# totgokhung123/Event-Retrival-In-Video-Learning-Transferable-Visual-Model-From-Supervised-Natural-Language

Measured on AMD Instinct MI355X. Metric: frames/sec embedded+ranked, ViT-B/32 224², 1/2/4/8 MI355X; R@1/5/10 parity, higher is better.
Workload: dtype bf16; 1 GPU; ViT-B/32 bf16, 10000 frames/GPU x 32 text queries, top-10 (BASELINE configs[1]); frames_per_gpu=10000, global_frames=10000, queries=32, k=10, image_chunk=10000, parallelism=dp1

## Files before the change

event-retrival-in-video-learning-transferable-visual-model-from-supervised-natural-language_amd/csrc/attention.hip:

```cpp
#include <algorithm>
#include <cstdlib>
#include <type_traits>

#include "common.hpp"
#include "internal.hpp"

namespace miclip {

namespace {


typedef short s16x4 __attribute__((ext_vector_type(4)));
typedef short s16x8 __attribute__((ext_vector_type(8)));

template <int V>
using Int = std::integral_constant<int, V>;

constexpr float sl2 = 0.125f * 1.4426950408889634f;
constexpr float RESCALE = 8.0f;

template <bool P16 = true>
__device__ __forceinline__ float group_max(float v) {
  if (P16) {
    const auto a = __builtin_amdgcn_permlane16_swap(__float_as_uint(v), __float_as_uint(v), false, false);
    v = fmaxf(__uint_as_float(a[0]), __uint_as_float(a[1]));
  }
  const auto b = __builtin_amdgcn_permlane32_swap(__float_as_uint(v), __float_as_uint(v), false, false);
  return fmaxf(__uint_as_float(b[0]), __uint_as_float(b[1]));
}
template <bool P16 = true>
__device__ __forceinline__ float group_sum(float v) {
  if (P16) {
    const auto a = __builtin_amdgcn_permlane16_swap(__float_as_uint(v), __float_as_uint(v), false, false);
    v = __uint_as_float(a[0]) + __uint_as_float(a[1]);
  }
  const auto b = __builtin_amdgcn_permlane32_swap(__float_as_uint(v), __float_as_uint(v), false, false);
  return __uint_as_float(b[0]) + __uint_as_float(b[1]);
}

template <class V, int N>
__device__ __forceinline__ void lazy_rescale(float& m, float& l, V (&o)[N], float cmu) {
  if (cmu > m + RESCALE) {
    const float alpha = __builtin_amdgcn_exp2f(m - cmu);
    l *= alpha;
#pragma unroll
    for (int i = 0; i < N; ++i) o[i] *= alpha;
    m = cmu;
  }
}

__device__ __forceinline__ void load_q16(const uint16_t* qb, int64_t ld, int tile, int S, int fr, int g, bf16x8 (&q)[2]) {
  const int qrow = min(tile * 16 + fr, S - 1);
#pragma unroll
  for (int s = 0; s < 2; ++s) q[s] = *(const bf16x8*)(qb + (int64_t)qrow * ld + 32 * s + 8 * g);
}

__device__ __forceinline__ s16x4 tr_read(const char* p) {
  return __builtin_amdgcn_ds_read_tr16_b64_v4i16((LDS_AS s16x4*)(LDS_AS char*)(uintptr_t)(const LDS_AS char*)p);
}
__device__ __forceinline__ bf16x8 vfrag(const char* p, int hi) {
  const s16x4 lo = tr_read(p);
  const s16x4 up = tr_read(p + hi);
  return __builtin_bit_cast(bf16x8, (s16x8)__builtin_shufflevector(lo, up, 0, 1, 2, 3, 4, 5, 6, 7));
}

struct AttnOut {
  uint16_t* out;
  uint8_t* q8;
  uint8_t* qs;
  int64_t rows_pad;
  int bseq, S, W, h;

  __device__ __forceinline__ void row16_bf16(int qrow, int g, const f32x4 (&o)[4], float inv) const {
    uint16_t* dst = out + ((int64_t)bseq * S + qrow) * W + h * 64 + 4 * g;
#pragma unroll
    for (int dt = 0; dt < 4; ++dt)
      *(uint2*)(dst + dt * 16) = make_uint2(pack_bf16x2(o[dt][0] * inv, o[dt][1] * inv),
                                            pack_bf16x2(o[dt][2] * inv, o[dt][3] * inv));
  }
  __device__ __forceinline__ void store16(int qrow, int g, const f32x4 (&o)[4], float inv) const {
    if (q8) {
      float amax = 0.f;
#pragma unroll
      for (int dt = 0; dt < 4; ++dt)
#pragma unroll
        for (int j = 0; j < 4; ++j) amax = fmaxf(amax, fabsf(o[dt][j] * inv));
      amax = fmaxf(amax, __shfl_xor(amax, 16, 64));
      amax = fmaxf(amax, __shfl_xor(amax, 32, 64));
      const int X = mx_block_exp(amax);
      const float scl = ldexpf(1.0f, -X);
      if (qrow < S) {
        const int64_t row = (int64_t)bseq * S + qrow;
        uint8_t* dst = q8 + row * W + h * 64 + 4 * g;
#pragma unroll
        for (int dt = 0; dt < 4; ++dt)
          *(uint32_t*)(dst + dt * 16) = mx_pack4(o[dt][0] * inv, o[dt][1] * inv, o[dt][2] * inv, o[dt][3] * inv, scl);
        if (g == 0) qs[mx_scale_index(row, h, rows_pad)] = (uint8_t)(X + 127);
      }
      return;
    }
    if (qrow < S) row16_bf16(qrow, g, o, inv);
  }
};

template <int SP>
__global__ __launch_bounds__(64) void attention_kernel(const uint16_t* __restrict__ qkv, uint16_t* __restrict__ out,
                                                       int S, int W, int H, int causal, int items) {
  constexpr int TS = SP + 8;
  __shared__ __attribute__((aligned(16))) uint16_t lds[64 * TS + 16 * TS];
  uint16_t* Vt = lds;
  uint16_t* Pw = lds + 64 * TS;
  const int item = blockIdx.x;
  if (item >= items) return;
  const int bseq = item / H, h = item % H;
  const int lane = threadIdx.x;
  const int64_t ld = 3 * (int64_t)W;
  const uint16_t* qb = qkv + (int64_t)bseq * S * ld + h * 64;
  const uint16_t* kb = qb + W;
  const uint16_t* vb = qb + 2 * W;

  for (int r0 = 0; r0 < SP; r0 += 8) {
    const int r = r0 + (lane & 7), ch = lane >> 3;
    uint4 v = make_uint4(0, 0, 0, 0);
    if (r < S) v = *(const uint4*)(vb + (int64_t)r * ld + ch * 8);
    const uint16_t* vv = (const uint16_t*)&v;
#pragma unroll
    for (int e = 0; e < 8; ++e) Vt[(ch * 8 + e) * TS + r] = vv[e];
  }

  constexpr int NKT = SP / 16;
  const float scale = 0.125f;
  const int fr = lane & 15, fk = 8 * (lane >> 4);
  const int nqt = (S + 15) / 16;
  for (int qt = 0; qt < nqt; ++qt) {
    const int64_t qrow = min(qt * 16 + fr, S - 1);
    bf16x8 qa[2];
#pragma unroll
    for (int s = 0; s < 2; ++s) qa[s] = *(const bf16x8*)(qb + qrow * ld + 32 * s + fk);
    f32x4 sc[NKT];
#pragma unroll
    for (int kt = 0; kt < NKT; ++kt) {
      const int64_t krow = min(kt * 16 + fr, S - 1);
      f32x4 c = {0.f, 0.f, 0.f, 0.f};
#pragma unroll
      for (int s = 0; s < 2; ++s) {
        const bf16x8 kf = *(const bf16x8*)(kb + krow * ld + 32 * s + fk);
        c = __builtin_amdgcn_mfma_f32_16x16x32_bf16(qa[s], kf, c, 0, 0, 0);
      }
      sc[kt] = c;
    }
#pragma unroll
    for (int j = 0; j < 4; ++j) {
      const int row = qt * 16 + 4 * (lane >> 4) + j;
      float m = -INFINITY;
#pragma unroll
      for (int kt = 0; kt < NKT; ++kt) {
        const int key = kt * 16 + fr;
        float v = sc[kt][j] * scale;
        if (key >= S || (causal && key > row)) v = -INFINITY;
        sc[kt][j] = v;
        m = fmaxf(m, v);
      }
#pragma unroll
      for (int o = 1; o < 16; o <<= 1) m = fmaxf(m, __shfl_xor(m, o, 64));
      float sum = 0.f;
#pragma unroll
      for (int kt = 0; kt < NKT; ++kt) {
        const float p = __expf(sc[kt][j] - m);
        sc[kt][j] = p;
        sum += p;
      }
#pragma unroll
      for (int o = 1; o < 16; o <<= 1) sum += __shfl_xor(sum, o, 64);
      const float inv = 1.0f / sum;
#pragma unroll
      for (int kt = 0; kt < NKT; ++kt) Pw[(4 * (lane >> 4) + j) * TS + kt * 16 + fr] = f2bf_hw(sc[kt][j] * inv);
    }
    asm volatile("s_waitcnt lgkmcnt(0)" ::: "memory");
    __builtin_amdgcn_wave_barrier();
    uint2 ov[4];
#pragma unroll
    for (int dt = 0; dt < 4; ++dt) {
      f32x4 o = {0.f, 0.f, 0.f, 0.f};
#pragma unroll
      for (int s = 0; s < SP / 32; ++s) {
        const bf16x8 va = *(const bf16x8*)(Vt + (dt * 16 + fr) * TS + 32 * s + fk);
        const bf16x8 pb = *(const bf16x8*)(Pw + fr * TS + 32 * s + fk);
        o = __builtin_amdgcn_mfma_f32_16x16x32_bf16(va, pb, o, 0, 0, 0);
      }
      ov[dt] = make_uint2(pack_bf16x2(o[0], o[1]), pack_bf16x2(o[2], o[3]));
    }
    const int row = qt * 16 + fr;
    if (row < S) {
      uint16_t* dst = out + ((int64_t)bseq * S + row) * W + h * 64 + 4 * (lane >> 4);
#pragma unroll
      for (int dt = 0; dt < 4; ++dt) *(uint2*)(dst + dt * 16) = ov[dt];
    }
    asm volatile("s_waitcnt lgkmcnt(0)" ::: "memory");
    __builtin_amdgcn_wave_barrier();
  }
}

template <int NT, int PP, int SLOTS, int HP = 1, bool PIPE = false, bool VB = false>
__device__ __forceinline__ void attention_flash_body(const uint16_t* __restrict__ qkv, uint16_t* __restrict__ out,
                                                     int S, int W, int H, int causal, uint8_t* __restrict__ q8,
                                                     uint8_t* __restrict__ qs, int64_t rows_pad, int items = 0) {
  static_assert(!PIPE || (NT == 1 && SLOTS == 1 && HP == 1), "PIPE: the single-chunk instance only");
  const bool q0only = causal & ATT_Q0_ONLY;
  causal &= ATT_CAUSAL;
  constexpr int KS = 72, VS = 68;
  const int NW = PP == 1 ? 8 : (int)(blockDim.x >> 6) / HP;
  __shared__ __attribute__((aligned(16))) uint16_t Ksh[HP][SLOTS][64 * KS];
  __shared__ __attribute__((aligned(16))) uint16_t Vsh[HP][SLOTS][64 * VS];
  const int hh = HP == 1 ? 0 : (int)(threadIdx.x >> 6) / NW;
  uint16_t(*Ks)[64 * KS] = Ksh[hh];
  uint16_t(*Vs)[64 * VS] = Vsh[hh];
  const int tid = threadIdx.x - hh * 64 * NW, lane = tid & 63, wave = tid >> 6;
  const int64_t ld = 3 * (int64_t)W;
#define FA_STAGE_LOAD(kb_, vb_, c, kr_, vr_)                                              \
  _Pragma("unroll") for (int i = 0; i < PP; ++i) {                                        \
    const int p_ = tid + i * 64 * NW, r_ = (c) * 64 + (p_ >> 3), ch_ = p_ & 7;            \
    kr_[i] = make_uint4(0, 0, 0, 0);                                                      \
    vr_[i] = make_uint4(0, 0, 0, 0);                                                      \
    if ((PP == 1 || p_ < 512) && r_ < S) {                                                \
      kr_[i] = *(const uint4*)((kb_) + (int64_t)r_ * ld + ch_ * 8);                       \
      vr_[i] = *(const uint4*)((vb_) + (int64_t)r_ * ld + ch_ * 8);                       \
    }                                                                                     \
  }
#define FA_STAGE_WRITE(slot)                                                              \
  _Pragma("unroll") for (int i = 0; i < PP; ++i) {                                        \
    const int p_ = tid + i * 64 * NW, r_ = p_ >> 3, ch_ = p_ & 7;                         \
    if (PP == 1 || p_ < 512) {                                                            \
      *(uint4*)(&Ks[slot][r_ * KS + ch_ * 8]) = kr[i];                                    \
      const uint16_t* vv_ = (const uint16_t*)&vr[i];                                      \
      _Pragma("unroll") for (int e = 0; e < 8; ++e) Vs[slot][(ch_ * 8 + e) * VS + r_] = vv_[e]; \
    }                                                                                     \
  }
  int item = blockIdx.x;
  bool first = true;
  uint4 kr_n[PP], vr_n[PP];
  bf16x8 qf_n[2];
  for (;;) {
  const int bseq = item / (H / HP), h = (item % (H / HP)) * HP + hh;
  const uint16_t* qb = qkv + (int64_t)bseq * S * ld + h * 64;
  const uint16_t* kb = qb + W;
  const uint16_t* vb = qb + 2 * W;
  const int nch = (S + 63) / 64, nqt = q0only ? 1 : (S + 15) / 16;
  const int fr = lane & 15, g = lane >> 4, fk = 8 * g;

  uint4 kr[PP], vr[PP];
  bf16x8 qf[NT][2];
  float m[NT], l[NT];
  f32x4 o[NT][4];
#pragma unroll
  for (int t = 0; t < NT; ++t) {
    const int qrow = min((wave + NW * t) * 16 + fr, S - 1);
#pragma unroll
    for (int s = 0; s < 2; ++s) qf[t][s] = (!PIPE || first) ? *(const bf16x8*)(qb + (int64_t)qrow * ld + 32 * s + fk) : qf_n[s];
    m[t] = -INFINITY;
    l[t] = 0.f;
#pragma unroll
    for (int dt = 0; dt < 4; ++dt) o[t][dt] = f32x4{0.f, 0.f, 0.f, 0.f};
  }
  if (!PIPE || first) {
    FA_STAGE_LOAD(kb, vb, 0, kr, vr);
  } else {
#pragma unroll
    for (int i = 0; i < PP; ++i) {
      kr[i] = kr_n[i];
      vr[i] = vr_n[i];
    }
  }
  FA_STAGE_WRITE(0);
  __syncthreads();
  if (PIPE && item + (int)gridDim.x < items) {
    const int nx = item + (int)gridDim.x;
    const uint16_t* nq = qkv + (int64_t)(nx / H) * S * ld + (nx % H) * 64;
    load_q16(nq, ld, wave, S, fr, g, qf_n);
    FA_STAGE_LOAD(nq + W, nq + 2 * W, 0, kr_n, vr_n);
  }

  for (int c = 0; c < nch; ++c) {
    const int slot = SLOTS == 1 ? 0 : (c & 1);
    if (SLOTS > 1 && c + 1 < nch) FA_STAGE_LOAD(kb, vb, c + 1, kr, vr);
    const int kvalid = min(64, S - c * 64);
    bf16x8 kf[4][2], vf[4][2];
#pragma unroll
    for (int kt = 0; kt < 4; ++kt)
#pragma unroll
      for (int s = 0; s < 2; ++s) kf[kt][s] = *(const bf16x8*)(&Ks[slot][(kt * 16 + fr) * KS + 32 * s + fk]);
    auto read_vf = [&]() {
#pragma unroll
      for (int dt = 0; dt < 4; ++dt)
#pragma unroll
        for (int s = 0; s < 2; ++s) {
          const uint16_t* vrow = &Vs[slot][(dt * 16 + fr) * VS + 32 * s + 4 * g];
          const uint2 lo = *(const uint2*)vrow;
          const uint2 hi = *(const uint2*)(vrow + 16);
          vf[dt][s] = __builtin_bit_cast(bf16x8, make_uint4(lo.x, lo.y, hi.x, hi.y));
        }
    };
    if (SLOTS > 1) read_vf();
#pragma unroll
    for (int t = 0; t < NT; ++t) {
      const int qt = wave + NW * t;
      if (qt >= nqt || (causal && c * 64 > qt * 16 + 15)) continue;
      const int qrow = qt * 16 + fr;
      f32x4 sc[4];
#pragma unroll
      for (int kt = 0; kt < 4; ++kt) {
        f32x4 acc = {0.f, 0.f, 0.f, 0.f};
        if (kt * 16 < kvalid) {
#pragma unroll
          for (int s = 0; s < 2; ++s) acc = __builtin_amdgcn_mfma_f32_16x16x32_bf16(kf[kt][s], qf[t][s], acc, 0, 0, 0);
        }
        sc[kt] = acc;
      }
      if (kvalid < 64 || (causal && (c + 1) * 64 > qt * 16)) {
#pragma unroll
        for (int kt = 0; kt < 4; ++kt)
#pragma unroll
          for (int j = 0; j < 4; ++j) {
            const int key = c * 64 + kt * 16 + 4 * g + j;
            if (key >= S || (causal && key > qrow)) sc[kt][j] = -INFINITY;
          }
      }
      float cm = fmaxf(fmaxf(fmaxf(sc[0][0], sc[0][1]), fmaxf(sc[0][2], sc[0][3])),
                       fmaxf(fmaxf(sc[1][0], sc[1][1]), fmaxf(sc[1][2], sc[1][3])));
      cm = fmaxf(cm, fmaxf(fmaxf(fmaxf(sc[2][0], sc[2][1]), fmaxf(sc[2][2], sc[2][3])),
                           fmaxf(fmaxf(sc[3][0], sc[3][1]), fmaxf(sc[3][2], sc[3][3]))));
      cm = group_max(cm);
      const float cmu = cm * sl2;
      if (cmu > m[t] + RESCALE) {
        const float alpha = __builtin_amdgcn_exp2f(m[t] - cmu);
        l[t] *= alpha;
#pragma unroll
        for (int dt = 0; dt < 4; ++dt) o[t][dt] *= alpha;
        m[t] = cmu;
      }
      const float mu = m[t];
      float ps[4];
#pragma unroll
      for (int kt = 0; kt < 4; ++kt) {
#pragma unroll
        for (int j = 0; j < 4; ++j) sc[kt][j] = __builtin_amdgcn_exp2f(fmaf(sc[kt][j], sl2, -mu));
        ps[kt] = (sc[kt][0] + sc[kt][1]) + (sc[kt][2] + sc[kt][3]);
      }
      l[t] += (ps[0] + ps[1]) + (ps[2] + ps[3]);
      if (SLOTS == 1) {
        __builtin_amdgcn_sched_barrier(0);
        read_vf();
        if (VB) asm volatile("s_waitcnt lgkmcnt(0)" ::: "memory");
      }
#pragma unroll
      for (int s = 0; s < 2; ++s) {
        if (s == 1 && kvalid <= 32) break;
        bf16x8 pb;
#pragma unroll
        for (int j = 0; j < 4; ++j) {
          pb[j] = (__bf16)sc[2 * s][j];
          pb[4 + j] = (__bf16)sc[2 * s + 1][j];
        }
#pragma unroll
        for (int dt = 0; dt < 4; ++dt) o[t][dt] = __builtin_amdgcn_mfma_f32_16x16x32_bf16(vf[dt][s], pb, o[t][dt], 0, 0, 0);
      }
    }
    if (SLOTS > 1 && c + 1 < nch) FA_STAGE_WRITE(slot ^ 1);
    __syncthreads();
  }
#undef FA_STAGE_LOAD
#undef FA_STAGE_WRITE

#pragma unroll
  for (int t = 0; t < NT; ++t) {
    const int qt = wave + NW * t;
    if (qt >= nqt) continue;
    AttnOut{out, q8, qs, rows_pad, bseq, S, W, h}.store16(qt * 16 + fr, g, o[t], 1.0f / group_sum(l[t]));
  }
  if (!PIPE) break;
  item += (int)gridDim.x;
  if (item >= items) break;
  first = false;
  }
}

template <int NT, int PP, int SLOTS = 2>
__global__ __launch_bounds__(512) void attention_flash_kernel(const uint16_t* __restrict__ qkv,
                                                                uint16_t* __restrict__ out, int S, int W, int H,
                                                                int causal, uint8_t* __restrict__ q8,
                                                                uint8_t* __restrict__ qs, int64_t rows_pad) {
  attention_flash_body<NT, PP, SLOTS>(qkv, out, S, W, H, causal, q8, qs, rows_pad);
}

#if MICLIP_AB
__global__ __launch_bounds__(256) __attribute__((amdgpu_waves_per_eu(6))) void attention_short_kernel(
    const uint16_t* __restrict__ qkv, uint16_t* __restrict__ out, int S, int W, int H, int causal,
    uint8_t* __restrict__ q8, uint8_t* __restrict__ qs, int64_t rows_pad) {
  attention_flash_body<1, 2, 1>(qkv, out, S, W, H, causal, q8, qs, rows_pad);
}

__global__ __launch_bounds__(256) void attention_pipe_kernel(const uint16_t* __restrict__ qkv, uint16_t* __restrict__ out,
                                                             int S, int W, int H, int causal, uint8_t* __restrict__ q8,
                                                             uint8_t* __restrict__ qs, int64_t rows_pad, int items) {
  attention_flash_body<1, 2, 1, 1, true>(qkv, out, S, W, H, causal, q8, qs, rows_pad, items);
}

__global__ __launch_bounds__(256) void attention_vb_kernel(const uint16_t* __restrict__ qkv, uint16_t* __restrict__ out,
                                                           int S, int W, int H, int causal, uint8_t* __restrict__ q8,
                                                           uint8_t* __restrict__ qs, int64_t rows_pad) {
  attention_flash_body<1, 2, 1, 1, false, true>(qkv, out, S, W, H, causal, q8, qs, rows_pad);
}

__global__ __launch_bounds__(512) __attribute__((amdgpu_waves_per_eu(6))) void attention_short2_kernel(
    const uint16_t* __restrict__ qkv, uint16_t* __restrict__ out, int S, int W, int H, int causal,
    uint8_t* __restrict__ q8, uint8_t* __restrict__ qs, int64_t rows_pad) {
  attention_flash_body<1, 2, 1, 2>(qkv, out, S, W, H, causal, q8, qs, rows_pad);
}
#endif


template <int NW, bool TT2 = true, bool SPLIT = false, bool SFIRST = false, bool QPF = false>
__global__ __launch_bounds__(NW * 64) void attention_res_kernel(const uint16_t* __restrict__ qkv,
                                                                uint16_t* __restrict__ out, int S, int W, int H,
                                                                uint8_t* __restrict__ q8, uint8_t* __restrict__ qs,
                                                                int64_t rows_pad) {
  extern __shared__ __attribute__((aligned(16))) char res_lds[];
  const int spad = (S + 31) & ~31;
  char* Kimg = res_lds;
  char* Vimg = res_lds + spad * 128;
  const int item = blockIdx.x;
  const int bseq = item / H, h = item % H;
  const int tid = threadIdx.x, lane = tid & 63;
  const int wave = __builtin_amdgcn_readfirstlane(tid >> 6);
  const int64_t ld = 3 * (int64_t)W;
  const uint16_t* qb = qkv + (int64_t)bseq * S * ld + h * 64;
  const uint16_t* kb = qb + W;
  const uint16_t* vb = qb + 2 * W;

  {
    const int nr8 = spad >> 3;
    const int slot = lane & 7;
    for (int i = wave; i < 2 * nr8; i += NW) {
      const bool isv = i >= nr8;
      const int i8 = isv ? i - nr8 : i;
      const int r = i8 * 8 + (lane >> 3);
      const int c = isv ? (slot ^ (((r >> 1) & 3) << 1)) : (slot ^ ((r >> 1) & 7));
      glds16((isv ? vb : kb) + (int64_t)min(r, S - 1) * ld + c * 8, (isv ? Vimg : Kimg) + i8 * 1024);
    }
  }

  const int nqt = (S + 15) / 16, nch = (S + 63) / 64;
  const int last_kvalid = S - (nch - 1) * 64;
  const int fr = lane & 15, g = lane >> 4;
  const int rk0 = fr * 128 + (((0 + g) ^ (fr >> 1)) << 4);
  const int rk1 = fr * 128 + (((4 + g) ^ (fr >> 1)) << 4);
  const int vq = (lane & 15) >> 2, vp = lane & 3;
  const int vx = (2 * g + (vq >> 1)) & 3;
  const int rvb = (4 * g + vq) * 128 + vp * 8;

  bf16x8 qn[2];
  if (QPF) load_q16(qb, ld, wave, S, fr, g, qn);
  asm volatile("s_waitcnt vmcnt(0)" ::: "memory");
  __syncthreads();

  auto tiles = [&](auto tt_c, int t0, int t1) {
    constexpr int TT = decltype(tt_c)::value;
    const int tq[2] = {t0, t1};
    bf16x8 qf[TT][2];
    if (QPF && TT == 1) {
      qf[0][0] = qn[0];
      qf[0][1] = qn[1];
      if (t0 + NW < (SPLIT ? nqt - 1 : nqt)) load_q16(qb, ld, t0 + NW, S, fr, g, qn);
    } else {
#pragma unroll
      for (int u = 0; u < TT; ++u) load_q16(qb, ld, tq[u], S, fr, g, qf[u]);
    }
    float m[TT], l[TT];
    f32x4 o[TT][4];
#pragma unroll
    for (int u = 0; u < TT; ++u) {
      m[u] = -INFINITY;
      l[u] = 0.f;
#pragma unroll
      for (int dt = 0; dt < 4; ++dt) o[u][dt] = f32x4{0.f, 0.f, 0.f, 0.f};
    }

    auto chunk = [&](auto nkt_c, auto mask_c, int c) {
      constexpr int NKT = decltype(nkt_c)::value;
      constexpr bool MASK = decltype(mask_c)::value;
      const char* kc = Kimg + c * 64 * 128;
      f32x4 sc[TT][NKT];
#pragma unroll
      for (int kt = 0; kt < NKT; ++kt) {
        const bf16x8 k0 = *(const bf16x8*)(kc + kt * 16 * 128 + rk0);
        const bf16x8 k1 = *(const bf16x8*)(kc + kt * 16 * 128 + rk1);
#pragma unroll
        for (int u = 0; u < TT; ++u) {
          const f32x4 acc = __builtin_amdgcn_mfma_f32_16x16x32_bf16(k0, qf[u][0], f32x4{0.f, 0.f, 0.f, 0.f}, 0, 0, 0);
          sc[u][kt] = __builtin_amdgcn_mfma_f32_16x16x32_bf16(k1, qf[u][1], acc, 0, 0, 0);
        }
      }
#pragma unroll
      for (int u = 0; u < TT; ++u) {
        if (MASK) {
#pragma unroll
          for (int kt = 0; kt < NKT; ++kt)
#pragma unroll
            for (int j = 0; j < 4; ++j)
              if (c * 64 + kt * 16 + 4 * g + j >= S) sc[u][kt][j] = -INFINITY;
        }
        float cm = fmaxf(fmaxf(sc[u][0][0], sc[u][0][1]), fmaxf(sc[u][0][2], sc[u][0][3]));
#pragma unroll
        for (int kt = 1; kt < NKT; ++kt)
          cm = fmaxf(cm, fmaxf(fmaxf(sc[u][kt][0], sc[u][kt][1]), fmaxf(sc[u][kt][2], sc[u][kt][3])));
        cm = group_max(cm);
        const float cmu = cm * sl2;
        lazy_rescale(m[u], l[u], o[u], cmu);
        float ps = 0.f;
#pragma unroll
        for (int kt = 0; kt < NKT; ++kt) {
#pragma unroll
          for (int j = 0; j < 4; ++j) sc[u][kt][j] = __builtin_amdgcn_exp2f(fmaf(sc[u][kt][j], sl2, -m[u]));
          ps += (sc[u][kt][0] + sc[u][kt][1]) + (sc[u][kt][2] + sc[u][kt][3]);
        }
        l[u] += ps;
      }
#pragma unroll
      for (int s2 = 0; s2 < (NKT + 1) / 2; ++s2) {
        bf16x8 pb[TT];
#pragma unroll
        for (int u = 0; u < TT; ++u)
#pragma unroll
          for (int j = 0; j < 4; ++j) {
            pb[u][j] = (__bf16)sc[u][2 * s2][j];
            pb[u][4 + j] = 2 * s2 + 1 < NKT ? (__bf16)sc[u][(2 * s2 + 1) < NKT ? 2 * s2 + 1 : 0][j] : (__bf16)0.f;
          }
        const char* vc = Vimg + (c * 64 + 32 * s2) * 128 + rvb;
#pragma unroll
        for (int dt = 0; dt < 4; ++dt) {
          const bf16x8 vf = vfrag(vc + ((dt ^ vx) << 5), 16 * 128);
#pragma unroll
          for (int u = 0; u < TT; ++u) o[u][dt] = __builtin_amdgcn_mfma_f32_16x16x32_bf16(vf, pb[u], o[u][dt], 0, 0, 0);
        }
      }
    };
    for (int c = 0; c < nch - 1; ++c) chunk(Int<4>{}, std::bool_constant<false>{}, c);
    {
      const int c = nch - 1;
      if (last_kvalid > 48) chunk(Int<4>{}, std::bool_constant<true>{}, c);
      else if (last_kvalid > 32) chunk(Int<3>{}, std::bool_constant<true>{}, c);
      else if (last_kvalid > 16) chunk(Int<2>{}, std::bool_constant<true>{}, c);
      else chunk(Int<1>{}, std::bool_constant<true>{}, c);
    }

#pragma unroll
    for (int u = 0; u < TT; ++u)
      AttnOut{out, q8, qs, rows_pad, bseq, S, W, h}.store16(tq[u] * 16 + fr, g, o[u], 1.0f / group_sum(l[u]));
  };
  auto split_part = [&]() __attribute__((always_inline)) {
    const int tl = nqt - 1, vr = S - 16 * tl;
    const int nkt = (S + 15) / 16;
    bf16x8 qf[2];
    load_q16(qb, ld, tl, S, fr, g, qf);
    float m = -INFINITY, l = 0.f;
    f32x4 o[4];
#pragma unroll
    for (int dt = 0; dt < 4; ++dt) o[dt] = f32x4{0.f, 0.f, 0.f, 0.f};
    for (int kt = wave; kt < nkt; kt += NW) {
      const int kb = kt * 16;
      const bf16x8 k0 = *(const bf16x8*)(Kimg + kb * 128 + rk0);
      const bf16x8 k1 = *(const bf16x8*)(Kimg + kb * 128 + rk1);
      f32x4 sc = __builtin_amdgcn_mfma_f32_16x16x32_bf16(k0, qf[0], f32x4{0.f, 0.f, 0.f, 0.f}, 0, 0, 0);
      sc = __builtin_amdgcn_mfma_f32_16x16x32_bf16(k1, qf[1], sc, 0, 0, 0);
#pragma unroll
      for (int j = 0; j < 4; ++j)
        if (kb + 4 * g + j >= S) sc[j] = -INFINITY;
      const float cm = group_max(fmaxf(fmaxf(sc[0], sc[1]), fmaxf(sc[2], sc[3])));
      const float cmu = cm * sl2;
      lazy_rescale(m, l, o, cmu);
#pragma unroll
      for (int j = 0; j < 4; ++j) sc[j] = __builtin_amdgcn_exp2f(fmaf(sc[j], sl2, -m));
      l += (sc[0] + sc[1]) + (sc[2] + sc[3]);
      bf16x8 pb;
#pragma unroll
      for (int j = 0; j < 4; ++j) {
        pb[j] = (__bf16)sc[j];
        pb[4 + j] = (__bf16)0.f;
      }
      const char* vc = Vimg + kb * 128 + rvb;
#pragma unroll
      for (int dt = 0; dt < 4; ++dt)
        o[dt] = __builtin_amdgcn_mfma_f32_16x16x32_bf16(vfrag(vc + ((dt ^ vx) << 5), 16 * 128), pb, o[dt], 0, 0, 0);
    }
    const float lt = group_sum(l);
    float* part = (float*)(res_lds + 2 * spad * 128);
    if (fr < vr) {
      float* pw = part + (wave * vr + fr) * 68;
#pragma unroll
      for (int dt = 0; dt < 4; ++dt)
#pragma unroll
        for (int j = 0; j < 4; ++j) pw[4 + dt * 16 + 4 * g + j] = o[dt][j];
      if (g == 0) {
        pw[0] = m;
        pw[1] = lt;
      }
    }
  };
  if (SPLIT && SFIRST) split_part();
  const int nfull = SPLIT ? nqt - 1 : nqt;
  for (int t = wave; t < nfull; t += 2 * NW) {
    if (TT2 && t + NW < nfull) tiles(Int<2>{}, t, t + NW);
    else {
      tiles(Int<1>{}, t, t);
      if (!TT2 && t + NW < nfull) tiles(Int<1>{}, t + NW, t + NW);
    }
  }
  if (SPLIT && !SFIRST) split_part();
  if (SPLIT) {
    const int tl = nqt - 1, vr = S - 16 * tl;
    float* part = (float*)(res_lds + 2 * spad * 128);
    __syncthreads();
    if (wave == 0 && fr < vr) {
      float M = -INFINITY;
#pragma unroll
      for (int w = 0; w < NW; ++w) M = fmaxf(M, part[(w * vr + fr) * 68]);
      float L = 0.f;
      f32x4 O[4];
#pragma unroll
      for (int dt = 0; dt < 4; ++dt) O[dt] = f32x4{0.f, 0.f, 0.f, 0.f};
#pragma unroll
      for (int w = 0; w < NW; ++w) {
        const float* pw = part + (w * vr + fr) * 68;
        const float sw = pw[0] == -INFINITY ? 0.f : __builtin_amdgcn_exp2f(pw[0] - M);
        L += pw[1] * sw;
#pragma unroll
        for (int dt = 0; dt < 4; ++dt)
#pragma unroll
          for (int j = 0; j < 4; ++j) O[dt][j] += pw[4 + dt * 16 + 4 * g + j] * sw;
      }
      AttnOut{out, q8, qs, rows_pad, bseq, S, W, h}.row16_bf16(tl * 16 + fr, g, O, 1.0f / L);
    }
  }
}

template <int N>
__device__ __forceinline__ void vm_wait_younger(int n) {
  if constexpr (N > 0) {
    if (n >= N) {
      asm volatile("s_waitcnt vmcnt(%0)" ::"n"(N) : "memory");
      return;
    }
    vm_wait_younger<N - 1>(n);
  } else {
    asm volatile("s_waitcnt vmcnt(0)" ::: "memory");
  }
}

template <int NW, bool TT2 = true, int ABL = 0, bool PH2 = false>
__global__ __launch_bounds__(NW * 64) void attention_r32_kernel(const uint16_t* __restrict__ qkv,
                                                                uint16_t* __restrict__ out, int S, int W, int H,
                                                                uint8_t* __restrict__ q8, uint8_t* __restrict__ qs,
                                                                int64_t rows_pad, int stagger_ticks) {
  extern __shared__ __attribute__((aligned(16))) char r32_lds[];
  const int spad = (S + 31) & ~31;
  char* Kimg = r32_lds;
  char* Vimg = r32_lds + spad * 128;
  const int item = blockIdx.x;
  const int bseq = item / H, head = item % H;
  const int tid = threadIdx.x, lane = tid & 63;
  const int wave = __builtin_amdgcn_readfirstlane(tid >> 6);
  const int64_t ld = 3 * (int64_t)W;
  const uint16_t* qb = qkv + (int64_t)bseq * S * ld + head * 64;
  const uint16_t* kb = qb + W;
  const uint16_t* vb = qb + 2 * W;

  if (stagger_ticks > 0 && (int)blockIdx.x < 256) {
    const int ph = (blockIdx.x >> 3) & 3;
    if (ph) {
      const uint64_t until = __builtin_amdgcn_s_memrealtime() + (uint64_t)ph * stagger_ticks;
      while (__builtin_amdgcn_s_memrealtime() < until) __builtin_amdgcn_s_sleep(8);
    }
  }
  const int nch = (S + 63) >> 6;
  const int nr8 = spad >> 3;
  const int c0 = PH2 ? max(1, nr8 >> 4) : nch;
  static_assert(!PH2 || (NW == 12 && !TT2), "attention_r32: the two-phase load's slot count assumes 12 waves");
  bf16x8 qf0[4];
  if (PH2) {
    const int qrow = min(wave * 32 + (lane & 31), S - 1);
#pragma unroll
    for (int s = 0; s < 4; ++s) qf0[s] = *(const bf16x8*)(qb + (int64_t)qrow * ld + 16 * s + 8 * (lane >> 5));
  }
  constexpr int NI2 = 14;
  const int h0 = 8 * c0;
  if (ABL != 2 && PH2) {
    const int slot = lane & 7;
    const int n1 = nr8 - h0;
#pragma unroll
    for (int k = 0; k < NI2; ++k) {
      const int g = min(wave + NW * k, 2 * nr8 - 1);
      const bool ph = g >= 2 * h0;
      const int j = ph ? g - 2 * h0 : g, cnt = ph ? n1 : h0;
      const bool isv = j >= cnt;
      const int i8 = (ph ? h0 : 0) + (isv ? j - cnt : j);
      const int rr = i8 * 8 + (lane >> 3);
      const int cc = isv ? (slot ^ (((rr >> 1) & 1) << 2)) : (slot ^ ((rr >> 1) & 7));
      glds16((isv ? vb : kb) + (int64_t)min(rr, S - 1) * ld + cc * 8, (isv ? Vimg : Kimg) + i8 * 1024);
    }
  }
  if (ABL != 2 && !PH2) {
    const int slot = lane & 7;
    for (int i = wave; i < 2 * nr8; i += NW) {
      const bool isv = i >= nr8;
      const int i8 = isv ? i - nr8 : i;
      const int rr = i8 * 8 + (lane >> 3);
      const int cc = isv ? (slot ^ (((rr >> 1) & 1) << 2)) : (slot ^ ((rr >> 1) & 7));
      glds16((isv ? vb : kb) + (int64_t)min(rr, S - 1) * ld + cc * 8, (isv ? Vimg : Kimg) + i8 * 1024);
    }
  }

  const int r = lane & 31, hh = lane >> 5;
  const int ksw = (r >> 1) & 7;
  const int i16 = lane & 15, gq = (lane >> 4) & 1, tq = i16 >> 2, tp = i16 & 3;
  const int vrow = (4 * hh + tq) * 128 + 8 * (tp & 1);
  const int vof0 = vrow + 16 * ((0 + 2 * gq + (tp >> 1)) ^ ((tq >> 1) << 2));
  const int vof1 = vrow + 16 * ((4 + 2 * gq + (tp >> 1)) ^ ((tq >> 1) << 2));
  const int nqb = (S + 31) >> 5;
  const int last_keys = S - (nch - 1) * 64;

  if (PH2) {
    const int n0 = 2 * h0 > wave ? (2 * h0 - wave + NW - 1) / NW : 0;
    vm_wait_younger<NI2>(NI2 - min(n0, NI2));
  } else {
    asm volatile("s_waitcnt vmcnt(0)" ::: "memory");
  }
  __syncthreads();

  auto blocks = [&](auto tt_c, int b0, int b1, bool first) {
    constexpr int TT = decltype(tt_c)::value;
    const int bq[2] = {b0, b1};
    bf16x8 qf[TT][4];
#pragma unroll
    for (int u = 0; u < TT; ++u) {
      const int qrow = min(bq[u] * 32 + r, S - 1);
#pragma unroll
      for (int s = 0; s < 4; ++s)
        qf[u][s] = PH2 && first ? qf0[s] : *(const bf16x8*)(qb + (int64_t)qrow * ld + 16 * s + 8 * hh);
    }
    float m[TT], l[TT];
    f32x16 o[TT][2];
#pragma unroll
    for (int u = 0; u < TT; ++u) {
      m[u] = -INFINITY;
      l[u] = 0.f;
#pragma unroll
      for (int i = 0; i < 16; ++i) o[u][0][i] = o[u][1][i] = 0.f;
    }

    auto chunk = [&](auto nkb_c, auto mask_c, int c) {
      constexpr int NKB = decltype(nkb_c)::value;
      constexpr bool MASK = decltype(mask_c)::value;
      f32x16 x[TT][NKB];
#pragma unroll
      for (int kt = 0; kt < NKB; ++kt) {
        const char* kp = Kimg + (c * 64 + kt * 32 + r) * 128;
        bf16x8 kf[4];
#pragma unroll
        for (int s = 0; s < 4; ++s) kf[s] = *(const bf16x8*)(kp + 16 * ((2 * s + hh) ^ ksw));
#pragma unroll
        for (int u = 0; u < TT; ++u) {
          f32x16 acc = __builtin_amdgcn_mfma_f32_32x32x16_bf16(kf[0], qf[u][0], f32x16{}, 0, 0, 0);
#pragma unroll
          for (int s = 1; s < 4; ++s) acc = __builtin_amdgcn_mfma_f32_32x32x16_bf16(kf[s], qf[u][s], acc, 0, 0, 0);
          x[u][kt] = acc;
        }
      }
#pragma unroll
      for (int u = 0; u < TT && ABL != 3; ++u) {
        if (MASK) {
#pragma unroll
          for (int kt = 0; kt < NKB; ++kt)
#pragma unroll
            for (int i = 0; i < 16; ++i)
              if (c * 64 + kt * 32 + c_row(i, hh) >= S) x[u][kt][i] = -INFINITY;
        }
        float cm = x[u][0][0];
#pragma unroll
        for (int kt = 0; kt < NKB; ++kt)
#pragma unroll
          for (int i = (kt ? 0 : 1); i < 16; ++i) cm = fmaxf(cm, x[u][kt][i]);
        cm = group_max<false>(cm);
        const float cmu = cm * sl2;
        lazy_rescale(m[u], l[u], o[u], cmu);
        float ps = 0.f;
#pragma unroll
        for (int kt = 0; kt < NKB; ++kt) {
#pragma unroll
          for (int i = 0; i < 16; ++i)
            x[u][kt][i] = ABL == 1 ? fmaf(x[u][kt][i], sl2, -m[u]) : __builtin_amdgcn_exp2f(fmaf(x[u][kt][i], sl2, -m[u]));
#pragma unroll
          for (int i = 0; i < 16; i += 4) ps += (x[u][kt][i] + x[u][kt][i + 1]) + (x[u][kt][i + 2] + x[u][kt][i + 3]);
        }
        l[u] += ps;
      }
#pragma unroll
      for (int kt = 0; kt < NKB; ++kt)
#pragma unroll
        for (int s = 0; s < 2; ++s) {
          const char* vp = Vimg + (c * 64 + kt * 32 + 16 * s) * 128;
          const bf16x8 v0 = vfrag(vp + vof0, 8 * 128);
          const bf16x8 v1 = vfrag(vp + vof1, 8 * 128);
#pragma unroll
          for (int u = 0; u < TT; ++u) {
            uint32_t pk[4];
#pragma unroll
            for (int j = 0; j < 4; ++j) pk[j] = pack_bf16x2(x[u][kt][8 * s + 2 * j], x[u][kt][8 * s + 2 * j + 1]);
            typedef uint32_t u32x4_t __attribute__((ext_vector_type(4)));
            const bf16x8 pb = __builtin_bit_cast(bf16x8, (u32x4_t){pk[0], pk[1], pk[2], pk[3]});
            o[u][0] = __builtin_amdgcn_mfma_f32_32x32x16_bf16(v0, pb, o[u][0], 0, 0, 0);
            o[u][1] = __builtin_amdgcn_mfma_f32_32x32x16_bf16(v1, pb, o[u][1], 0, 0, 0);
          }
        }
    };
    for (int c = 0; c < nch - 1; ++c) {
      if (PH2 && first && c == c0) {
        asm volatile("s_waitcnt vmcnt(0)" ::: "memory");
        __syncthreads();
      }
      chunk(Int<2>{}, std::bool_constant<false>{}, c);
    }
    if (PH2 && first && c0 >= nch - 1) {
      asm volatile("s_waitcnt vmcnt(0)" ::: "memory");
      __syncthreads();
    }
    if (last_keys > 32) chunk(Int<2>{}, std::bool_constant<true>{}, nch - 1);
    else chunk(Int<1>{}, std::bool_constant<true>{}, nch - 1);

#pragma unroll
    for (int u = 0; u < TT; ++u) {
      const float inv = 1.0f / group_sum<false>(l[u]);
      const int qrow = bq[u] * 32 + r;
      if (q8) {
        float amax = 0.f;
#pragma unroll
        for (int db = 0; db < 2; ++db)
#pragma unroll
          for (int i = 0; i < 16; ++i) amax = fmaxf(amax, fabsf(o[u][db][i] * inv));
        amax = group_max<false>(amax);
        const int X = mx_block_exp(amax);
        const float scl = ldexpf(1.0f, -X);
        if (qrow < S) {
          const int64_t row = (int64_t)bseq * S + qrow;
          uint8_t* dst = q8 + row * W + head * 64 + 4 * hh;
#pragma unroll
          for (int db = 0; db < 2; ++db)
#pragma unroll
            for (int t = 0; t < 4; ++t)
              *(uint32_t*)(dst + 32 * db + 8 * t) = mx_pack4(o[u][db][4 * t] * inv, o[u][db][4 * t + 1] * inv,
                                                             o[u][db][4 * t + 2] * inv, o[u][db][4 * t + 3] * inv, scl);
          if (hh == 0) qs[mx_scale_index(row, head, rows_pad)] = (uint8_t)(X + 127);
        }
        continue;
      }
      if (qrow < S) {
        uint16_t* dst = out + ((int64_t)bseq * S + qrow) * W + head * 64 + 4 * hh;
#pragma unroll
        for (int db = 0; db < 2; ++db)
#pragma unroll
          for (int t = 0; t < 4; ++t)
            *(uint2*)(dst + 32 * db + 8 * t) = make_uint2(pack_bf16x2(o[u][db][4 * t] * inv, o[u][db][4 * t + 1] * inv),
                                                          pack_bf16x2(o[u][db][4 * t + 2] * inv, o[u][db][4 * t + 3] * inv));
      }
    }
  };
  if (TT2) {
    for (int b = wave; b < nqb; b += 2 * NW) {
      if (b + NW < nqb) blocks(Int<2>{}, b, b + NW, false);
      else blocks(Int<1>{}, b, b, false);
    }
  } else {
    if (PH2 && wave >= nqb) {
      asm volatile("s_waitcnt vmcnt(0)" ::: "memory");
      __syncthreads();
    }
    for (int b = wave; b < nqb; b += NW) blocks(Int<1>{}, b, b, b == wave);
  }
}

}

template <auto KERNEL>
using Kern = std::integral_constant<decltype(KERNEL), KERNEL>;

hipError_t attention(const uint16_t* qkv, uint16_t* out, int B, int S, int W, int flags, hipStream_t s, uint8_t* q8,
                     uint8_t* qs) {
  const int H = W / 64;
  const int items = B * H;
  if (items <= 0) return hipSuccess;
  if (S > 640) return hipErrorInvalidValue;

#if MICLIP_AB
  const bool one_wave = (flags & ATT_ONE_WAVE) && S <= 96 && !q8;
#else
  if (flags & ATT_ONE_WAVE) return hipErrorNotSupported;
  constexpr bool one_wave = false;
#endif
  const bool stream = flags & ATT_STREAM;
  const int q0 = flags & ATT_Q0_ONLY;
  const int causal = flags & ATT_CAUSAL;
  const int64_t rows_pad = ((int64_t)B * S + 1) & ~1;
  const size_t res_lds = 2 * (size_t)((S + 31) & ~31) * 128;

#if MICLIP_AB
  if (!one_wave && !stream && S <= 64) {
    const int sw = ab_env_int("MICLIP_ATTN_SHORT", 0);
    if (sw == 5 || sw / 10 == 5) {
      const int per = sw == 5 ? 4 : sw % 10;
      const int gp = std::min(items, cu_count() * (per > 0 ? per : 5));
      return launch_kernel(attention_pipe_kernel, gp, 256, s, qkv, out, S, W, H, causal, q8, qs, rows_pad, items);
    }
    switch (sw) {
      case 6:
        return launch_kernel(attention_vb_kernel, items, 256, s, qkv, out, S, W, H, causal | q0, q8, qs, rows_pad);
      case 2:
        if (H % 2 == 0)
          return launch_kernel(attention_short2_kernel, items / 2, 512, s, qkv, out, S, W, H, causal, q8, qs, rows_pad);
        [[fallthrough]];
      case 3:
        return launch_kernel(attention_short_kernel, items, 256, s, qkv, out, S, W, H, causal, q8, qs, rows_pad);
      case 1:
        if (!causal)
          return launch_kernel<attention_res_kernel<4, false>>(items, 256, res_lds, s, qkv, out, S, W, H, q8, qs, rows_pad);
        break;
      default: break;
    }
  }
#endif

  if (!one_wave && !stream && !causal && S > 64) {
    int var = ab_env_int("MICLIP_ATTN_VAR", 0);
    if (var < 1 || var > 14) var = S > 320 ? 5 : 1;
    const int vr = S - 16 * ((S + 15) / 16 - 1);
    if (var == 11 || ((var == 12 || var == 13) && !(vr <= 4 && !q8))) var = 1;
    auto res = [&](auto k, int threads, size_t lds) {
      return launch_kernel<decltype(k)::value>(items, threads, lds, s, qkv, out, S, W, H, q8, qs, rows_pad);
    };
    auto r32 = [&](auto k, int threads, int stagger_ticks) {
      return launch_kernel<decltype(k)::value>(items, threads, res_lds, s, qkv, out, S, W, H, q8, qs, rows_pad,
                                               stagger_ticks);
    };
    switch (var) {
      case 1: return res(Kern<attention_res_kernel<8, false>>{}, 512, res_lds);
      case 5: return r32(Kern<attention_r32_kernel<12, false>>{}, 768, 0);
#if MICLIP_AB
      case 2: return res(Kern<attention_res_kernel<8, true>>{}, 512, res_lds);
      case 3: return res(Kern<attention_res_kernel<16, false>>{}, 1024, res_lds);
      case 4: return r32(Kern<attention_r32_kernel<8, true>>{}, 512, 0);
      case 6:
      case 7:
        return r32(Kern<attention_r32_kernel<12, false>>{}, 768, (var - 5) * (S * S / 378));
      case 8: return r32(Kern<attention_r32_kernel<12, false, 2>>{}, 768, 0);
      case 10: return r32(Kern<attention_r32_kernel<12, false, 0, true>>{}, 768, 0);
      case 12: return res(Kern<attention_res_kernel<8, false, true>>{}, 512, res_lds + (size_t)8 * vr * 68 * 4);
      case 13: return res(Kern<attention_res_kernel<8, false, true, true>>{}, 512, res_lds + (size_t)8 * vr * 68 * 4);
      case 14: return res(Kern<attention_res_kernel<8, false, false, false, true>>{}, 512, res_lds);
      default: return r32(Kern<attention_r32_kernel<12, false, 1>>{}, 768, 0);
#else
      default: return hipErrorNotSupported;
#endif
    }
  }

#if MICLIP_AB
  if (one_wave)
    return with_value<32, 64, 96>(std::max(32, (S + 31) & ~31), [&](auto sp) {
      return launch_kernel(attention_kernel<decltype(sp)::value>, items, 64, s, qkv, out, S, W, H, causal, items);
    });
#endif

  const int nqt = (S + 15) / 16;
  if (nqt <= 4)
    return launch_kernel(attention_flash_kernel<1, 2, 1>, items, 256, s, qkv, out, S, W, H, causal | q0, q8, qs, rows_pad);
  return with_value<1, 2, 3, 4, 5>((nqt + 7) / 8, [&](auto nt) {
    return launch_kernel(attention_flash_kernel<decltype(nt)::value, 1>, items, 512, s, qkv, out, S, W, H, causal, q8, qs,
                         rows_pad);
  });
}

}
```

Measured before the change: 118,900 frames/s.

## Add persistent producer/consumer ring attention kernel for short sequences

Adds a persistent attention kernel for S<=64 non-causal attention. One or two loader waves stream Q/K/V tiles into a multi-slot LDS ring using global_load_lds, and the remaining waves consume them with MFMA softmax-attention, handing slots back through LDS full/freed flags. Output is staged through LDS so the global stores are coalesced. It becomes the default path when there are at least 4 items per CU, which is meant to hide load latency and cut launch and occupancy overhead, at the cost of spin-wait flag synchronisation and fewer compute waves.

Result: no change. 119,800 frames/s (median of 6 runs) (+0.7%).

```diff
diff --git a/event-retrival-in-video-learning-transferable-visual-model-from-supervised-natural-language_amd/csrc/attention.hip b/event-retrival-in-video-learning-transferable-visual-model-from-supervised-natural-language_amd/csrc/attention.hip
--- a/event-retrival-in-video-learning-transferable-visual-model-from-supervised-natural-language_amd/csrc/attention.hip
+++ b/event-retrival-in-video-learning-transferable-visual-model-from-supervised-natural-language_amd/csrc/attention.hip
@@ -887,6 +887,238 @@
   }
 }
 
+constexpr int RING_MAT = 64 * 128;
+constexpr int RING_SLOT = 3 * RING_MAT;
+constexpr int RING_MAX_SLOTS = 6;
+constexpr int RING_WAVES = 8;
+constexpr int RING_FLAGS = 64;
+constexpr int RING_STAGE = 16 * 128;
+constexpr size_t ring_lds_bytes(int nslot) { return (size_t)nslot * RING_SLOT + RING_FLAGS + (RING_WAVES - 1) * RING_STAGE; }
+static_assert(2 * RING_MAX_SLOTS * 4 <= RING_FLAGS && ring_lds_bytes(RING_MAX_SLOTS) <= 160 * 1024, "attention_ring: LDS");
+struct RingCfg {
+  int nslot, nl, nc, look, rev;
+  int probe;
+  int direct;
+  int nts;
+};
+
+__device__ __forceinline__ uint32_t ring_flag_read(const uint32_t* p) {
+  uint32_t v;
+  const uint32_t addr = (uint32_t)(uintptr_t)(const LDS_AS uint32_t*)p;
+  asm volatile("ds_read_b32 %0, %1\n\ts_waitcnt lgkmcnt(0)" : "=v"(v) : "v"(addr) : "memory");
+  return __builtin_amdgcn_readfirstlane(v);
+}
+__device__ __forceinline__ void ring_flag_write(uint32_t* p, uint32_t v) {
+  const uint32_t addr = (uint32_t)(uintptr_t)(LDS_AS uint32_t*)p;
+  asm volatile("ds_write_b32 %0, %1\n\ts_waitcnt lgkmcnt(0)" ::"v"(addr), "v"(v) : "memory");
+}
+
+template <int R8, bool NT>
+__global__ __launch_bounds__(RING_WAVES * 64) void attention_ring_kernel(const uint16_t* __restrict__ qkv,
+                                                                         uint16_t* __restrict__ out, int S, int W, int H,
+                                                                         int q0, uint8_t* __restrict__ q8,
+                                                                         uint8_t* __restrict__ qs, int64_t rows_pad, int items,
+                                                                         RingCfg cfg) {
+  static_assert(R8 >= 1 && R8 <= 8, "attention_ring: S <= 64");
+  constexpr int NQT = (R8 + 1) / 2;
+  constexpr int Q0_OPS = R8 < 2 ? R8 : 2;
+  constexpr int OPS = 3 * R8, OPS_Q0 = 2 * R8 + Q0_OPS;
+  constexpr int YCAP = VM_MAX / OPS < 3 ? VM_MAX / OPS : 3;
+  constexpr int AUX = NT ? 2 : 0;
+  extern __shared__ __attribute__((aligned(16))) char ring_lds[];
+  const int nslot = cfg.nslot, nl = cfg.nl, nc = cfg.nc;
+  const int look = min(cfg.look, YCAP);
+  uint32_t* full = (uint32_t*)(ring_lds + nslot * RING_SLOT);
+  uint32_t* freed = full + RING_MAX_SLOTS;
+  const int tid = threadIdx.x, lane = tid & 63;
+  const int wave = __builtin_amdgcn_readfirstlane(tid >> 6);
+  const int64_t ld = 3 * (int64_t)W;
+  const int G = gridDim.x;
+  const int nk = ((int)blockIdx.x < items) ? (items - (int)blockIdx.x + G - 1) / G : 0;
+  auto item_of = [&](int k) {
+    const int i = (int)blockIdx.x + k * G;
+    return cfg.rev ? items - 1 - i : i;
+  };
+
+  if (tid < 2 * RING_MAX_SLOTS) full[tid] = 0;
+  if constexpr (R8 < 8) {
+    constexpr int PAD16 = (64 - 8 * R8) * 8;
+    for (int i = tid; i < nslot * 2 * PAD16; i += RING_WAVES * 64) {
+      const int sl = i / (2 * PAD16), r = i - sl * 2 * PAD16;
+      const int mat = 1 + r / PAD16, p = r % PAD16;
+      *(uint4*)(ring_lds + sl * RING_SLOT + mat * RING_MAT + 8 * R8 * 128 + p * 16) = make_uint4(0, 0, 0, 0);
+    }
+  }
+  __syncthreads();
+
+  if (wave < nl) {
+    const int slotc = lane & 7, rl = lane >> 3;
+    auto issue = [&](int k) __attribute__((always_inline)) {
+      const int item = item_of(k);
+      const int bseq = item / H, h = item - bseq * H;
+      const uint16_t* qb = qkv + (int64_t)bseq * S * ld + h * 64;
+      char* sl = ring_lds + (k % nslot) * RING_SLOT;
+      int vm = 0;
+#if MICLIP_VMCHECK
+#define MI_VM_ISSUED(n) (vm += (n))
+#else
+#define MI_VM_ISSUED(n) ((void)0)
+#endif
+      auto rows8 = [&](int mat, int i) __attribute__((always_inline)) {
+        const int r = i * 8 + rl;
+        const int c = mat == 2 ? (slotc ^ (((r >> 1) & 3) << 1)) : (slotc ^ ((r >> 1) & 7));
+        __builtin_amdgcn_global_load_lds((const GLB_AS void*)(qb + mat * W + (int64_t)min(r, S - 1) * ld + c * 8),
+                                         (LDS_AS void*)(sl + mat * RING_MAT + i * 1024), 16, 0, AUX);
+        MI_VM_ISSUED(1);
+      };
+#pragma unroll
+      for (int i = 0; i < R8; ++i) rows8(1, i);
+#pragma unroll
+      for (int i = 0; i < R8; ++i) rows8(2, i);
+      if (q0) {
+#pragma unroll
+        for (int i = 0; i < Q0_OPS; ++i) rows8(0, i);
+        if (MICLIP_VMCHECK) vm_count_check<OPS_Q0>(vm);
+      } else {
+#pragma unroll
+        for (int i = 0; i < R8; ++i) rows8(0, i);
+        if (MICLIP_VMCHECK) vm_count_check<OPS>(vm);
+      }
+#undef MI_VM_ISSUED
+    };
+    auto publish = [&](int k, int younger) __attribute__((always_inline)) {
+      if (q0) vm_wait_stages<OPS_Q0, YCAP>(younger);
+      else vm_wait_stages<OPS, YCAP>(younger);
+      ring_flag_write(&full[k % nslot], (uint32_t)(k + 1));
+    };
+    int issued = 0, k = wave;
+    for (; k < nk; k += nl) {
+      if (k >= nslot) {
+        const uint32_t want = (uint32_t)(k - nslot + 1);
+        while (ring_flag_read(&freed[k % nslot]) != want) __builtin_amdgcn_s_sleep(1);
+      }
+      issue(k);
+      if (issued >= look) publish(k - look * nl, look);
+      ++issued;
+    }
+    for (int j = min(issued, look) - 1; j >= 0; --j) publish(k - nl - j * nl, j);
+    return;
+  }
+  if (wave >= nl + nc) return;
+
+  const int fr = lane & 15, g = lane >> 4;
+  const int vq = fr >> 2, vp = lane & 3;
+  const int vx = (2 * g + (vq >> 1)) & 3;
+  const int rvb = (4 * g + vq) * 128 + vp * 8;
+  const int nqt = q0 ? 1 : NQT;
+  char* stage = ring_lds + nslot * RING_SLOT + RING_FLAGS + (wave - nl) * RING_STAGE;
+  for (int k = wave - nl; k < nk; k += nc) {
+    const int slot = k % nslot;
+    while (ring_flag_read(&full[slot]) != (uint32_t)(k + 1)) __builtin_amdgcn_s_sleep(1);
+    if (cfg.probe == 1) {
+      ring_flag_write(&freed[slot], (uint32_t)(k + 1));
+      continue;
+    }
+    const char* Qi = ring_lds + slot * RING_SLOT;
+    const char* Ki = Qi + RING_MAT;
+    const char* Vi = Qi + 2 * RING_MAT;
+    bf16x8 qf[NQT][2], kf[NQT][2], vf[4][2];
+#pragma unroll
+    for (int t = 0; t < NQT; ++t) {
+      const int qrow = min(t * 16 + fr, S - 1);
+#pragma unroll
+      for (int s = 0; s < 2; ++s) qf[t][s] = *(const bf16x8*)(Qi + qrow * 128 + (((4 * s + g) ^ ((qrow >> 1) & 7)) << 4));
+    }
+#pragma unroll
+    for (int kt = 0; kt < NQT; ++kt)
+#pragma unroll
+      for (int s = 0; s < 2; ++s) kf[kt][s] = *(const bf16x8*)(Ki + (kt * 16 + fr) * 128 + (((4 * s + g) ^ (fr >> 1)) << 4));
+#pragma unroll
+    for (int s = 0; s < (R8 > 4 ? 2 : 1); ++s)
+#pragma unroll
+      for (int dt = 0; dt < 4; ++dt) vf[dt][s] = vfrag(Vi + 32 * s * 128 + rvb + ((dt ^ vx) << 5), 16 * 128);
+    asm volatile("s_waitcnt lgkmcnt(0)" ::: "memory");
+    ring_flag_write(&freed[slot], (uint32_t)(k + 1));
+
+    const int item = item_of(k);
+    const int bseq = item / H, h = item - bseq * H;
+#pragma unroll
+    for (int t = 0; t < NQT; ++t) {
+      if (t >= nqt) break;
+      float m = -INFINITY, l = 0.f;
+      f32x4 o[4];
+#pragma unroll
+      for (int dt = 0; dt < 4; ++dt) o[dt] = f32x4{0.f, 0.f, 0.f, 0.f};
+      f32x4 sc[4];
+#pragma unroll
+      for (int kt = 0; kt < 4; ++kt) {
+        f32x4 acc = {0.f, 0.f, 0.f, 0.f};
+        if (kt < NQT) {
+#pragma unroll
+          for (int s = 0; s < 2; ++s) acc = __builtin_amdgcn_mfma_f32_16x16x32_bf16(kf[kt < NQT ? kt : 0][s], qf[t][s], acc, 0, 0, 0);
+        }
+        sc[kt] = acc;
+      }
+      if (S < 64) {
+#pragma unroll
+        for (int kt = 0; kt < 4; ++kt)
+#pragma unroll
+          for (int j = 0; j < 4; ++j)
+            if (kt * 16 + 4 * g + j >= S) sc[kt][j] = -INFINITY;
+      }
+      float cm = fmaxf(fmaxf(fmaxf(sc[0][0], sc[0][1]), fmaxf(sc[0][2], sc[0][3])),
+                       fmaxf(fmaxf(sc[1][0], sc[1][1]), fmaxf(sc[1][2], sc[1][3])));
+      cm = fmaxf(cm, fmaxf(fmaxf(fmaxf(sc[2][0], sc[2][1]), fmaxf(sc[2][2], sc[2][3])),
+                           fmaxf(fmaxf(sc[3][0], sc[3][1]), fmaxf(sc[3][2], sc[3][3]))));
+      cm = group_max(cm);
+      const float cmu = cm * sl2;
+      lazy_rescale(m, l, o, cmu);
+      const float mu = m;
+      float ps[4];
+#pragma unroll
+      for (int kt = 0; kt < 4; ++kt) {
+#pragma unroll
+        for (int j = 0; j < 4; ++j) sc[kt][j] = __builtin_amdgcn_exp2f(fmaf(sc[kt][j], sl2, -mu));
+        ps[kt] = (sc[kt][0] + sc[kt][1]) + (sc[kt][2] + sc[kt][3]);
+      }
+      l += (ps[0] + ps[1]) + (ps[2] + ps[3]);
+#pragma unroll
+      for (int s = 0; s < (R8 > 4 ? 2 : 1); ++s) {
+        bf16x8 pb;
+#pragma unroll
+        for (int j = 0; j < 4; ++j) {
+          pb[j] = (__bf16)sc[2 * s][j];
+          pb[4 + j] = (__bf16)sc[2 * s + 1][j];
+        }
+#pragma unroll
+        for (int dt = 0; dt < 4; ++dt) o[dt] = __builtin_amdgcn_mfma_f32_16x16x32_bf16(vf[dt][s], pb, o[dt], 0, 0, 0);
+      }
+      const float inv = 1.0f / group_sum(l);
+      if (cfg.probe == 2) continue;
+      if (q8 || cfg.direct) {
+        AttnOut{out, q8, qs, rows_pad, bseq, S, W, h}.store16(t * 16 + fr, g, o, inv);
+        continue;
+      }
+#pragma unroll
+      for (int dt = 0; dt < 4; ++dt)
+        *(uint2*)(stage + fr * 128 + (((2 * dt + (g >> 1)) ^ (fr & 7)) << 4) + (g & 1) * 8) =
+            make_uint2(pack_bf16x2(o[dt][0] * inv, o[dt][1] * inv), pack_bf16x2(o[dt][2] * inv, o[dt][3] * inv));
+#pragma unroll
+      for (int hf = 0; hf < 2; ++hf) {
+        const int r = hf * 8 + (lane >> 3), c = lane & 7;
+        const uint4 v = *(const uint4*)(stage + r * 128 + ((c ^ (r & 7)) << 4));
+        const int qrow = t * 16 + r;
+        uint4* dst = (uint4*)(out + ((int64_t)bseq * S + qrow) * W + h * 64 + c * 8);
+        if (qrow < S) {
+          typedef uint32_t u32x4_nt __attribute__((ext_vector_type(4)));
+          if (cfg.nts) __builtin_nontemporal_store(__builtin_bit_cast(u32x4_nt, v), (u32x4_nt*)dst);
+          else *dst = v;
+        }
+      }
+    }
+  }
+}
+
 }
 
 template <auto KERNEL>
@@ -906,14 +1138,42 @@
   constexpr bool one_wave = false;
 #endif
   const bool stream = flags & ATT_STREAM;
-  const int q0 = flags & ATT_Q0_ONLY;
+  const int q0 = (flags & ATT_Q0_ONLY) | (ab_env_int("MICLIP_ATTN_Q0", 0) ? (int)ATT_Q0_ONLY : 0);
   const int causal = flags & ATT_CAUSAL;
   const int64_t rows_pad = ((int64_t)B * S + 1) & ~1;
   const size_t res_lds = 2 * (size_t)((S + 31) & ~31) * 128;
 
+  const int sw = (!one_wave && !stream && S <= 64) ? ab_env_int("MICLIP_ATTN_SHORT", 0) : 0;
+  if (!one_wave && !stream && !causal && S <= 64 && (sw == 0 || sw == 7 || sw == 8)) {
+    constexpr int RING_MIN_ITEMS = 4;
+    const int cus = cu_count(), cap = ab_env_int("MICLIP_ATTN_RING_WGS", 0);
+    if (sw != 0 || items >= RING_MIN_ITEMS * cus) {
+      const int grid = std::min(items, cap > 0 ? std::min(cap, cus) : cus);
+      RingCfg cfg;
+      cfg.nslot = std::clamp(ab_env_int("MICLIP_ATTN_RING_SLOTS", RING_MAX_SLOTS), 2, RING_MAX_SLOTS);
+      cfg.nl = std::clamp(ab_env_int("MICLIP_ATTN_RING_LOADERS", 1), 1, 2);
+      cfg.nc = RING_WAVES - cfg.nl;
+      cfg.look = std::clamp(ab_env_int("MICLIP_ATTN_RING_LOOK", 1), 0, (cfg.nslot - 2) / cfg.nl);
+      cfg.rev = sw == 8;
+      cfg.probe = ab_env_int("MICLIP_ATTN_RING_PROBE", 0);
+      cfg.direct = ab_env_int("MICLIP_ATTN_RING_STORE", 1) == 0;
+      cfg.nts = ab_env_int("MICLIP_ATTN_RING_NTS", 0);
+      [[maybe_unused]] const bool nt = ab_env_int("MICLIP_ATTN_RING_NT", 0) != 0;
+      return with_value<1, 2, 3, 4, 5, 6, 7, 8>((S + 7) / 8, [&](auto r8) {
+        auto go = [&](auto k) {
+          return launch_kernel<decltype(k)::value>(grid, RING_WAVES * 64, ring_lds_bytes(cfg.nslot), s, qkv, out, S, W, H, q0, q8,
+                                                   qs, rows_pad, items, cfg);
+        };
+#if MICLIP_AB
+        if (nt) return go(Kern<attention_ring_kernel<decltype(r8)::value, true>>{});
+#endif
+        return go(Kern<attention_ring_kernel<decltype(r8)::value, false>>{});
+      });
+    }
+  }
+
 #if MICLIP_AB
   if (!one_wave && !stream && S <= 64) {
-    const int sw = ab_env_int("MICLIP_ATTN_SHORT", 0);
     if (sw == 5 || sw / 10 == 5) {
       const int per = sw == 5 ? 4 : sw % 10;
       const int gp = std::min(items, cu_count() * (per > 0 ? per : 5));
```
